# SkyTNT/midi-model

Hardware: AMD Instinct MI355X
Metric: MIDI events/sec, training step (fwd+bwd+clip+AdamW), tv2o-medium, seq=2048 (higher is better)
Workload: dtype bf16; 1 GPU; tv2o-medium bf16 training step, per-GPU batch 16 x 2048 events x 8 tokens (BASELINE.json configs[1]); random-init weights, synthetic events; global_batch=16, seq_len=2048, parallelism=dp1, accumulate_grad_batches=1, optimizer=AdamW bf16-true + global-norm clip 1.0

## Files before the change

include/midihip.h:

```cpp
#ifndef MIDIHIP_H
#define MIDIHIP_H
#include <stdint.h>
#ifdef __cplusplus
extern "C" {
#endif

#define MH_F32 0
#define MH_BF16 1

#define MH_OK 0
#define MH_ERR_ARG (-1)
#define MH_ERR_LAUNCH (-2)
#define MH_ERR_UNSUPPORTED (-3)

const char* mh_last_error(void);
int mh_version(void);
int mh_ab_builds(void);
int mh_set_option(const char* name, int value);
int mh_get_option(const char* name);

int mh_gemm_nt(const void* A, int64_t lda, const void* B, int64_t ldb, void* C, int64_t ldc, const void* R,
               int64_t ldr, int64_t M, int64_t N, int64_t K, float alpha, float beta, int dtype, int splitk,
               void* workspace, void* stream);
int mh_gemm(const void* A, int64_t lda, int transA, const void* B, int64_t ldb, int transB, void* C, int64_t ldc,
            const void* R, int64_t ldr, int64_t M, int64_t N, int64_t K, float alpha, float beta, int dtype, int splitk,
            void* workspace, void* stream);
int mh_gemm_swiglu(const void* A, int64_t lda, const void* W, int64_t ldw, void* GU, int64_t ldgu, void* ACT,
                   int64_t ldact, int64_t M, int64_t I, int64_t K, int dtype, void* stream);
int mh_gemm_rope(const void* A, int64_t lda, const void* W, int64_t ldw, void* C, int64_t ldc, const void* table,
                 int64_t npos, int64_t S, int64_t pos0, int head_dim, int64_t M, int64_t N, int64_t K, int dtype, void* stream);
int mh_gemm_dswiglu(const void* A, int64_t lda, const void* B, int64_t ldb, const void* GU, int64_t ldgu, void* DGU,
                    int64_t lddgu, int64_t M, int64_t I, int64_t K, int dtype, void* stream);
int mh_gemm_rowss(const void* A, int64_t lda, const void* B, int64_t ldb, void* C, int64_t ldc, const void* R, int64_t ldr,
                  float* rowss, int64_t M, int64_t N, int64_t K, int dtype, void* stream);
int mh_row_rstd(const void* x, int64_t ldx, const float* parts, int nparts, int64_t M, int D, float eps, float* rstd, int dtype,
                void* stream);
int mh_gemm_rope_scaled(const void* A, int64_t lda, const void* W, int64_t ldw, void* C, int64_t ldc, const void* table,
                        int64_t npos, int64_t S, int64_t pos0, int head_dim, const float* rowscale, int64_t M, int64_t N, int64_t K,
                        int dtype, void* stream);
int mh_gemm_swiglu_scaled(const void* A, int64_t lda, const void* W, int64_t ldw, void* GU, int64_t ldgu, void* ACT, int64_t ldact,
                          const float* rowscale, int64_t M, int64_t I, int64_t K, int dtype, void* stream);
int mh_gemm_nt_scaled(const void* A, int64_t lda, const void* B, int64_t ldb, void* C, int64_t ldc, const float* rowscale, int64_t M,
                      int64_t N, int64_t K, int dtype, void* stream);
int mh_gemm_dswiglu_scaled(const void* A, int64_t lda, const void* B, int64_t ldb, const void* GU, int64_t ldgu, void* DGU,
                           int64_t lddgu, const float* rowscale, int64_t M, int64_t I, int64_t K, int dtype, void* stream);
int mh_splitk_fold_blocks(int64_t M);
int mh_gemm_splitk_reduce_fold(const void* workspace, void* C, int64_t ldc, const void* R, int64_t ldr, int64_t M, int64_t N,
                               int splitk, float alpha, float beta, const void* wnorm, const void* W, int64_t ldw, float* colpart,
                               int dtype, void* stream);
int mh_rmsnorm_bwd_folded(const void* x, const float* rstd, const void* t, const void* dres, void* dx, int64_t M, int D, int dtype,
                          void* stream);
int mh_scale_cols(const void* W, int64_t ldw, const void* w, void* out, int64_t ldo, int64_t Nr, int K, int dtype, void* stream);
int mh_scale_cols_batched(const int64_t* jobs, int njobs, int K, int dtype, void* stream);
int mh_gemm_splitk_reduce(const void* workspace, void* C, int64_t ldc, const void* R, int64_t ldr, int64_t M,
                          int64_t N, int splitk, float alpha, float beta, int dtype, void* stream);
#define MH_SKINNY_PLAIN 0
#define MH_SKINNY_GATEUP 1
int mh_gemm_skinny(const void* A, int64_t lda, const void* W, int64_t ldw, void* C, int64_t ldc, const void* R,
                   int64_t ldr, int mode, float norm_eps, const int64_t* row_ids, const int64_t* res_ids, int64_t M,
                   int64_t N, int64_t K, int dtype, void* stream);
int mh_gemm_skinny_wide(const void* A, int64_t lda, const void* W, int64_t ldw, void* C, int64_t ldc, const void* R,
                        int64_t ldr, int mode, float norm_eps, const int64_t* row_ids, const int64_t* res_ids, int64_t M,
                        int64_t N, int64_t K, int dtype, void* stream);
int mh_transpose(const void* in, int64_t ldi, void* out, int64_t ldo, int64_t rows, int64_t cols, int dtype,
                 void* stream);

int mh_embed_sum_fwd(const int64_t* tok, const void* table, void* out, int64_t M, int T, int64_t V, int D,
                     int dtype, void* stream);
int mh_concat_tok_fwd(const void* hidden, const int64_t* tok, int64_t ldtok, const void* table, void* out,
                      int64_t M, int T, int64_t V, int D, int dtype, void* stream);
int mh_embed_scatter_bwd(const int64_t* tok, int64_t ldtok, int T, const void* dout, int rows_per_m, int jstride,
                         int j0, float* dtable_f32, int64_t M, int64_t V, int D, int64_t pad_id, int dtype,
                         void* stream);
int mh_embed_segment_bwd(const int64_t* src_rows, const int64_t* seg_start, const void* dout, int64_t ld,
                         float* dtable_f32, int64_t V, int D, int64_t n_occ, int64_t pad_id, int dtype, void* stream);
int mh_embed_segment_sum(const int64_t* src_rows, const int64_t* seg_start, const void* rows, int64_t ld, float* sum_f32,
                         int64_t ldsum, int64_t V, int D, int64_t n_occ, int dtype, void* stream);
int mh_embed_split_hi_lo(const float* s, void* hi, void* lo, int64_t n, int dtype, void* stream);
int mh_embed_table_norm_bwd(const void* t_hi, const void* t_lo, const void* e, const float* rstd, float* acc32, int64_t V, int D,
                            int64_t pad_id, int dtype, void* stream);
int mh_token_segments_chunk(void);
int mh_token_segments(const int64_t* tok, int64_t ldtok, int64_t n_rows, int n_cols, int64_t V, int64_t row_mul,
                      int64_t col_mul, int64_t add, int64_t* src_rows, int64_t* seg_start, int32_t* work, void* stream);
int mh_cast_from_f32(const float* src, void* dst, int64_t n, int accumulate, int dtype, void* stream);
int mh_copy_rows(const void* src, int64_t src_ld, void* dst, int64_t dst_ld, int64_t M, int D, int accumulate,
                 int dtype, void* stream);

int mh_collate_windows(const int16_t* tokens, int64_t n_events, const int64_t* win_start, const int64_t* win_len,
// ... 133 lines not shown
```

midi-model_amd/csrc/common.h:

```cpp
#pragma once
#include <hip/hip_runtime.h>
#include <stdint.h>

#include "../../include/midihip.h"

#define MH_WAVE 64

typedef __bf16 bf16;
typedef __attribute__((ext_vector_type(8))) __bf16 bf16x8;
typedef __attribute__((ext_vector_type(4))) __bf16 bf16x4;
typedef __attribute__((ext_vector_type(4))) float f32x4;
typedef __attribute__((ext_vector_type(16))) float f32x16;
typedef __attribute__((address_space(3))) void lds_void_t;
typedef __attribute__((address_space(1))) const void glb_void_t;

void mh_set_error(const char* fmt, ...);
#define MH_REQUIRE(cond, ...)            \
  do {                                   \
    if (!(cond)) {                       \
      mh_set_error(__VA_ARGS__);         \
      return MH_ERR_ARG;                 \
    }                                    \
  } while (0)
#define MH_LAUNCH_CHECK()                                            \
// ... 137 lines not shown
  auto take = [&](uint32_t ohi, uint32_t olo) {
    const bool better = ohi > hi || (ohi == hi && olo > lo);
    hi = better ? ohi : hi;
    lo = better ? olo : lo;
  };
  take(dpp_move_u<0xB1>(hi), dpp_move_u<0xB1>(lo));
  take(dpp_move_u<0x4E>(hi), dpp_move_u<0x4E>(lo));
  take(dpp_move_u<0x141>(hi), dpp_move_u<0x141>(lo));
  take(dpp_move_u<0x140>(hi), dpp_move_u<0x140>(lo));
  {
    auto a = __builtin_amdgcn_permlane16_swap(hi, hi, false, false);
    auto b = __builtin_amdgcn_permlane16_swap(lo, lo, false, false);
    hi = a[0];
    lo = b[0];
    take(a[1], b[1]);
  }
  {
    auto a = __builtin_amdgcn_permlane32_swap(hi, hi, false, false);
    auto b = __builtin_amdgcn_permlane32_swap(lo, lo, false, false);
    hi = a[0];
    lo = b[0];
    take(a[1], b[1]);
  }
  return ((uint64_t)hi << 32) | lo;
}

__device__ inline int lds_swz(int row) { return (((row >> 1) & 1) << 2) | (((row >> 2) & 1) << 1) | ((row >> 3) & 1); }
__device__ inline int lds_tile_off(int row, int chunk) { return row * 128 + ((chunk ^ lds_swz(row)) << 4); }

__device__ inline void glds16(const void* src, void* lds_rows8) {
  __builtin_amdgcn_global_load_lds((glb_void_t*)src, (lds_void_t*)lds_rows8, 16, 0, 0);
}

__device__ inline void gemm_tile_of(int idx, int tiles_m, int tiles_n, int GM, int& tm, int& tn) {
  const int width = GM * tiles_n;
  const int gid = idx / width;
  const int first = gid * GM;
  const int gsize = (tiles_m - first < GM) ? tiles_m - first : GM;
  const int rem = idx - gid * width;
  tn = rem / gsize;
  tm = first + (rem - tn * gsize);
}

__device__ inline int pi32(int i) { return (i & ~12) | ((i & 4) << 1) | ((i & 8) >> 1); }
```

midi-model_amd/csrc/gemm_pp256.hip:

```cpp
#include <limits.h>

#include <type_traits>

#include "common.h"

namespace {

__device__ __attribute__((aligned(16))) char g_zero16[16];

constexpr int QBM = 256, QBN = 256, QBK = 32;
constexpr int OP_BYTES = 256 * 64;
constexpr int STAGE_BYTES = 2 * OP_BYTES;
constexpr int NSTAGE = 4;
constexpr int LDS_BYTES = NSTAGE * STAGE_BYTES;
constexpr int NWAVE = 8;
constexpr int NI = 2;

typedef __attribute__((ext_vector_type(4))) short s16x4_t;

__device__ inline int tswz(int krow) { return (krow & 3) | ((krow >> 1) & 4); }
__device__ inline int xswz(int row) { return (0x1230 >> (((row >> 2) & 3) * 4)) & 3; }

struct StageCtx {
  const bf16* p[NI];
// ... 265 lines not shown
    for (int p = 0; p < 2; ++p) {
      stamp();
      if (2 * t + p > 0) mfma_phase(p ^ 1);
      else stamp();
      bar();
      stamp();
      load_slot(t, p, steady);
      wait_next(2 * t + p, steady);
      bar();
    }
  };

#pragma unroll
  for (int s = 0; s < LA; ++s)
    if (s < nreg) issue(s);
  if (nt > 0) wait_out((nreg < LA ? nreg : LA) - need(0));
  bar();
  mark(253);
  const int nsteady = nt > 2 ? nt - 2 : 0;
  if (grp == 0) {
    for (int t = 0; t < nsteady; ++t) tile_g0(t, std::true_type{});
    for (int t = nsteady; t < nt; ++t) tile_g0(t, std::false_type{});
  } else {
    for (int t = 0; t < nsteady; ++t) tile_g1(t, std::true_type{});
    for (int t = nsteady; t < nt; ++t) tile_g1(t, std::false_type{});
    if (nt > 0) mfma_phase(1);
  }
  mark(254);
  if constexpr (TL) {
    asm volatile("s_waitcnt lgkmcnt(0)" ::: "memory");
  }
}

template <bool TA, bool TB, int ABL, int EPI, int ML, int NRM>
__global__ __launch_bounds__(512, 2) void gemm_pp256_kernel(const bf16* __restrict__ A, int64_t lda,
                                                            const bf16* __restrict__ B, int64_t ldb, bf16* C, int64_t ldc,
                                                            const bf16* R, int64_t ldr, int64_t M, int64_t N, int64_t K,
                                                            float alpha, float beta, int tiles_n, int nwg,
                                                            int64_t k_per_split, float* __restrict__ ws,
                                                            const void* __restrict__ zero16, float* aux, int lean_epi) {
  static_assert(NRM == 0 || (ML == 1 && ABL == 0 && !TA && (!TB || (EPI == 1 && NRM == 2))), "the norm forms ride on the K-step-64 loops only");
  static_assert(NRM != 1 || EPI == 0, "sum-of-squares partials come out of the plain epilogue");
  extern __shared__ __attribute__((aligned(16))) char smem[];
  const int tid = threadIdx.x, lane = tid & 63;
  const int wave = __builtin_amdgcn_readfirstlane(tid >> 6);
  const int grp = wave >> 2;
  const int wn = wave & 3;

  const int nitems = nwg * (int)gridDim.z;
  const int lin = blockIdx.x + nwg * (int)blockIdx.z;
  const int q = nitems >> 3, r8 = nitems & 7, xcd = lin & 7;
  const int item = (xcd < r8 ? xcd * (q + 1) : r8 * (q + 1) + (xcd - r8) * q) + (lin >> 3);
  const int zslice = item / nwg;
  int tm, tn;
  gemm_tile_of(item - zslice * nwg, nwg / tiles_n, tiles_n, 4, tm, tn);
  const int64_t m0 = (int64_t)tm * QBM, n0 = (int64_t)tn * (EPI == 2 ? 128 : QBN);

  const int64_t kbeg = (int64_t)zslice * k_per_split;
  const int64_t kend = (kbeg + k_per_split < K) ? kbeg + k_per_split : K;

  f32x4 acc[4][8];
#pragma unroll
  for (int a = 0; a < 4; ++a)
#pragma unroll
    for (int b = 0; b < 8; ++b) acc[a][b] = f32x4{0.f, 0.f, 0.f, 0.f};
  const int fi = lane & 15, fg = lane >> 4;
  auto bar = [&]() {
    __builtin_amdgcn_sched_barrier(0);
    __builtin_amdgcn_s_barrier();
    __builtin_amdgcn_sched_barrier(0);
  };

  if constexpr (ML >= 1) {
    if constexpr (NRM == 2) {
      if (wave == 0) {
        const int64_t r = m0 + lane * 4;
        glds16((r + 4 <= M) ? (const void*)(aux + r) : zero16, smem + LDS_BYTES);
      }
    }
    p8_main_loop<EPI, ABL, TB>(smem, A, lda, B, ldb, M, N, m0, n0, kbeg, kend, wave, lane, zero16, acc);
    if constexpr ((ABL & 128) != 0) {
      __syncthreads();
      if (blockIdx.x == 0 && blockIdx.z == 0)
        for (int i = tid; i < P8_DBG_BYTES / 8; i += 512)
          reinterpret_cast<uint64_t*>(ws)[i] = reinterpret_cast<const uint64_t*>(smem + 2 * P8_BUF)[i];
      __syncthreads();
    }
  } else {
// ... 410 lines not shown
          const bf16x2 lo = __builtin_convertvector(f32x2{a4[0], a4[1]}, bf16x2), hi2 = __builtin_convertvector(f32x2{a4[2], a4[3]}, bf16x2);
          f32x4 r4;
          r4[0] = (float)lo[0];
          r4[1] = (float)lo[1];
          r4[2] = (float)hi2[0];
          r4[3] = (float)hi2[1];
          *reinterpret_cast<f32x4*>(wreg + row * 256 + ((ch ^ (row & 15)) << 4)) = r4;
        }
      if (half == 0) request(1);
#pragma unroll
      for (int i = 0; i < 8; ++i) {
        const int row = i * 8 + lrow;
        const f32x4 lo = *reinterpret_cast<const f32x4*>(wreg + row * 256 + (((2 * c) ^ (row & 15)) << 4));
        const f32x4 hi = *reinterpret_cast<const f32x4*>(wreg + row * 256 + (((2 * c + 1) ^ (row & 15)) << 4));
        const int64_t m = m0 + grp * 128 + half * 64 + row;
        float v[8] = {lo[0], lo[1], lo[2], lo[3], hi[0], hi[1], hi[2], hi[3]};
        if (rot) {
          const int pc = c ^ 4;
          const f32x4 plo = *reinterpret_cast<const f32x4*>(wreg + row * 256 + (((2 * pc) ^ (row & 15)) << 4));
          const f32x4 phi = *reinterpret_cast<const f32x4*>(wreg + row * 256 + (((2 * pc + 1) ^ (row & 15)) << 4));
          const float pv[8] = {plo[0], plo[1], plo[2], plo[3], phi[0], phi[1], phi[2], phi[3]};
          float cf[8], sf[8];
          expand8_bf16(cv[i], cf);
          expand8_bf16(sv[i], sf);
#pragma unroll
          for (int e = 0; e < 8; ++e) v[e] = __builtin_fmaf(v[e], cf[e], pv[e] * sf[e]);
        }
        if (m >= M || n + 8 > N) continue;
        __builtin_nontemporal_store(cvt8_bf16(v), reinterpret_cast<bf16x8*>(C + m * ldc + n));
      }
    }
    return;
  }
  const bool use_r = (R != nullptr && beta != 0.f);
  const bool line_ok = !partial && (ldc & 7) == 0 && ((uintptr_t)C & 15) == 0 &&
                       (!use_r || ((ldr & 7) == 0 && ((uintptr_t)R & 15) == 0));
  if (lean_epi && line_ok && m0 + QBM <= M && n0 + QBN <= N && ldc < (1 << 22) && ldr < (1 << 22)) {
    char* wreg = smem + wave * 16384;
    const int lrow = lane >> 3, c = lane & 7;
    const __amdgpu_buffer_rsrc_t rc = tile_rsrc(C + m0 * ldc + n0 + wn * 64, (255 * ldc + 64) * 2);
    const __amdgpu_buffer_rsrc_t rr = tile_rsrc(use_r ? R + m0 * ldr + n0 + wn * 64 : nullptr, use_r ? (255 * ldr + 64) * 2 : 0);
    const unsigned vo_c = (unsigned)(((grp * 128 + lrow) * (int)ldc + c * 8) * 2), so_c = (unsigned)ldc * 16u;
    const unsigned vo_r = (unsigned)(((grp * 128 + lrow) * (int)ldr + c * 8) * 2), so_r = (unsigned)ldr * 16u;
    float* auxp = nullptr;
    if constexpr (NRM == 1) auxp = aux + ((n0 + wn * 64) >> 6) * M + m0 + grp * 128 + lrow;
    auto turn = [&](auto with_r) {
    constexpr bool use_r = decltype(with_r)::value;
    bf16x8 rv[2][8];
    if (use_r) {
#pragma unroll
      for (int half = 0; half < 2; ++half)
#pragma unroll
        for (int i = 0; i < 8; ++i)
          rv[half][i] = as_bf16x8(__builtin_amdgcn_raw_buffer_load_b128(rr, vo_r, (unsigned)(half * 8 + i) * so_r, 0));
    }
#pragma unroll
    for (int half = 0; half < 2; ++half) {
#pragma unroll
      for (int fmh = 0; fmh < 4; ++fmh)
#pragma unroll
        for (int fn = 0; fn < 4; ++fn) {
          const int row = fmh * 16 + fi, ch = fn * 4 + fg;
          f32x4 t4 = acc[fn][half * 4 + fmh];
          if constexpr (NRM == 2) t4 *= rs[half * 4 + fmh];
          *reinterpret_cast<f32x4*>(wreg + row * 256 + ((ch ^ (row & 15)) << 4)) = t4;
        }
// ... 125 lines not shown
          *reinterpret_cast<f32x4*>(dst) = v;
        } else {
          for (int e = 0; e < 4 && n + e < N; ++e) dst[e] = v[e];
        }
        continue;
      }
      if (vec_ok && n + 3 < N) {
        if (R != nullptr && beta != 0.f) {
          bf16x4 rv = *reinterpret_cast<const bf16x4*>(R + m * ldr + n);
#pragma unroll
          for (int e = 0; e < 4; ++e) v[e] = alpha * v[e] + beta * (float)rv[e];
        } else {
#pragma unroll
          for (int e = 0; e < 4; ++e) v[e] = alpha * v[e];
        }
        bf16x4 o;
#pragma unroll
        for (int e = 0; e < 4; ++e) o[e] = (bf16)v[e];
        *reinterpret_cast<bf16x4*>(C + m * ldc + n) = o;
      } else {
        for (int e = 0; e < 4 && n + e < N; ++e) {
          float x = alpha * v[e];
          if (R != nullptr && beta != 0.f) x += beta * (float)R[m * ldr + n + e];
          C[m * ldc + n + e] = (bf16)x;
        }
      }
    }
  }
}

}
extern thread_local int g_mh_gemm_lean_epi;
namespace {
template <bool TA, bool TB, int ABL, int EPI = 0, int ML = 0, int NRM = 0>
int launch_one(const void* A, int64_t lda, const void* B, int64_t ldb, void* C, int64_t ldc, const void* R, int64_t ldr,
               int64_t M, int64_t N, int64_t K, float alpha, float beta, int splitk, void* workspace, hipStream_t st,
               float* aux = nullptr) {
  constexpr int LDSB = LDS_BYTES + ((ABL & 128) ? P8_DBG_BYTES : 0) + (NRM == 2 ? 1024 : 0);
  constexpr int MAX_DEV = 64;
  static void* zero16_of[MAX_DEV] = {};
  static bool attr_set_of[MAX_DEV] = {};
  int dev = 0;
  if (hipGetDevice(&dev) != hipSuccess || dev < 0 || dev >= MAX_DEV) {
    mh_set_error("gemm_pp256: no current device (or ordinal %d beyond %d)", dev, MAX_DEV - 1);
    return MH_ERR_LAUNCH;
  }
  void* zero16 = __atomic_load_n(&zero16_of[dev], __ATOMIC_ACQUIRE);
  if (zero16 == nullptr) {
    if (hipGetSymbolAddress(&zero16, HIP_SYMBOL(g_zero16)) != hipSuccess) {
      mh_set_error("gemm_pp256: hipGetSymbolAddress(g_zero16) failed");
      return MH_ERR_LAUNCH;
    }
    __atomic_store_n(&zero16_of[dev], zero16, __ATOMIC_RELEASE);
  }
  if (!__atomic_load_n(&attr_set_of[dev], __ATOMIC_ACQUIRE)) {
    hipError_t e = hipFuncSetAttribute(reinterpret_cast<const void*>(&gemm_pp256_kernel<TA, TB, ABL, EPI, ML, NRM>),
                                       hipFuncAttributeMaxDynamicSharedMemorySize, LDSB);
    if (e != hipSuccess) {
      mh_set_error("gemm_pp256: cannot raise dynamic LDS to %d bytes: %s", LDSB, hipGetErrorString(e));
      return MH_ERR_LAUNCH;
    }
    __atomic_store_n(&attr_set_of[dev], true, __ATOMIC_RELEASE);
  }
  const int64_t tiles_m = (M + QBM - 1) / QBM, tiles_n = (EPI == 2) ? N / 256 : (N + QBN - 1) / QBN;
  const int nwg = (int)(tiles_m * tiles_n);
  constexpr int KSTEP = (ML == 1) ? 64 : QBK;
  const int64_t kps = ((K + splitk - 1) / splitk + KSTEP - 1) / KSTEP * KSTEP;
  dim3 grid(nwg, 1, splitk);
  gemm_pp256_kernel<TA, TB, ABL, EPI, ML, NRM><<<grid, 512, LDSB, st>>>((const bf16*)A, lda, (const bf16*)B, ldb, (bf16*)C, ldc,
                                                          (const bf16*)R, ldr, M, N, K, alpha, beta, (int)tiles_n, nwg, kps,
                                                          (float*)workspace, zero16, aux, g_mh_gemm_lean_epi);
  MH_LAUNCH_CHECK();
  return MH_OK;
}

}

extern thread_local int g_mh_gemm_ablate;
extern thread_local int g_mh_gemm_k64;

int mh_gemm_pp256_bf16(const void* A, int64_t lda, int ta, const void* B, int64_t ldb, int tb, void* C, int64_t ldc,
                       const void* R, int64_t ldr, int64_t M, int64_t N, int64_t K, float alpha, float beta, int splitk,
                       void* workspace, hipStream_t st) {
#define MH_PP(TA_, TB_, ABL_) \
  return launch_one<TA_, TB_, ABL_>(A, lda, B, ldb, C, ldc, R, ldr, M, N, K, alpha, beta, splitk, workspace, st)
#ifndef MH_AB_BUILDS
  MH_REQUIRE(g_mh_gemm_ablate == 0, "gemm: option gemm_ablate = %d selects a micro-benchmark build, which is only in the A/B test "
             "library (libmidihip_ab.so)", g_mh_gemm_ablate);
#else
  MH_REQUIRE(g_mh_gemm_ablate != 128 || (workspace != nullptr && splitk == 1), "gemm_ablate 128 (timeline) needs a workspace and splitk 1");
  MH_REQUIRE(!(g_mh_gemm_k64 && !ta && !tb) || g_mh_gemm_ablate == 0 || g_mh_gemm_ablate == 1 || g_mh_gemm_ablate == 4 ||
                 g_mh_gemm_ablate == 128 || g_mh_gemm_ablate == 64,
             "gemm_ablate %d is not built for the K-step-64 main loop (set gemm_k64 = 0 for the K-step-32 ablations)", g_mh_gemm_ablate);
  if (ta == tb && g_mh_gemm_ablate && !(g_mh_gemm_k64 && !ta)) {
#define MH_AB(X_) \
  case X_:        \
    if (ta) MH_PP(true, true, X_); \
    MH_PP(false, false, X_);
    switch (g_mh_gemm_ablate) { MH_AB(1) MH_AB(3) MH_AB(4) MH_AB(5) MH_AB(8) MH_AB(12) MH_AB(32) default: break; }
#undef MH_AB
  }
  if (g_mh_gemm_ablate == 64) {
    if (ta && tb) MH_PP(true, true, 64);
    if (ta) MH_PP(true, false, 64);
    if (tb) MH_PP(false, true, 64);
    MH_PP(false, false, 64);
  }
#endif
  if (ta && tb) MH_PP(true, true, 0);
  if (ta) MH_PP(true, false, 0);
  if (tb && g_mh_gemm_k64 == 1)
// ... 68 lines not shown
```

midi-model_amd/engine.py:

```python
from __future__ import annotations

import math
from dataclasses import dataclass, field
from typing import Callable, List, NamedTuple, Optional

import os

import torch

from . import ops, tokfirst


@dataclass
class StackSpec:
    name: str
    D: int
    H: int
    I: int
    L: int
    eps: float
    theta: float
    kind: str

    @property
# ... 270 lines not shown
        ops.swiglu_bwd(keep.gu, da, dgu)
        del da
    linear_wgrad(dx, a, lg.wd, accumulate)
    del a
    dh2 = _empty((M, D), dx)
    ops.gemm_nt(dgu, lw.wgu, dh2, tb=True)
    linear_wgrad(dgu, keep.h2, lg.wgu, accumulate)
    del dgu
    dx2 = _empty((M, D), dx)
    ops.rmsnorm_bwd(keep.x2, lw.n2, keep.rstd2, dh2, dx, dx2, lg.n2, accumulate)
    do = dh2
    ops.gemm_nt(dx2, lw.wo, do, tb=True)
    linear_wgrad(dx2, keep.o, lg.wo, accumulate)
    dqkv = _empty((M, 3 * D), dx)
    if seqs is not None:
        ops.attn_bwd_seqs(keep.qkv, keep.o, do, keep.lse, dqkv, seqs, H, spec.scale, rope.cos, rope.sin)
    elif spec.kind == "event":
        ops.attn_bwd(keep.qkv, keep.o, do, keep.lse, dqkv, nseq, slen, H, spec.scale, rope.cos, rope.sin)
    else:
        ops.tokattn_bwd(keep.qkv, do, dqkv, nseq, slen, H, spec.scale, rope.cos, rope.sin)
    dh1 = do
    ops.gemm_nt(dqkv, lw.wqkv, dh1, tb=True)
    linear_wgrad(dqkv, keep.h1, lg.wqkv, accumulate)
    del dqkv
    ops.rmsnorm_bwd(keep.x, lw.n1, keep.rstd1, dh1, dx2, dx, lg.n1, accumulate)
    return dx


def layer_backward_folded(spec: StackSpec, lw: LayerTensors, lg: LayerTensors, fold, keep: LayerSaved, dx: torch.Tensor, nseq: int,
                          slen: int, rope: RopeTable, accumulate: bool, seqs=None) -> torch.Tensor:
    M, D = dx.shape
    H = spec.H
    wq_n, wgu_n = fold
    dx2, do = _folded_mlp_o_backward(spec, lw, lg, wgu_n, keep, dx, accumulate)
    dz1 = _empty((M, 3 * D), dx)
    if seqs is not None:
        ops.attn_bwd_seqs(keep.qkv, keep.o, do, keep.lse, dz1, seqs, H, spec.scale, rope.cos, rope.sin, rowscale=keep.rstd1)
    elif spec.kind == "event":
        ops.attn_bwd(keep.qkv, keep.o, do, keep.lse, dz1, nseq, slen, H, spec.scale, rope.cos, rope.sin, rowscale=keep.rstd1)
    else:
        ops.tokattn_bwd(keep.qkv, do, dz1, nseq, slen, H, spec.scale, rope.cos, rope.sin, rowscale=keep.rstd1)
    t1 = do
    ops.gemm_nt(dz1, wq_n, t1, tb=True)
    ops.wgrad_folded(dz1, keep.x, lg.wqkv, lw.n1, lw.wqkv, lg.n1, accumulate)
    del dz1
    ops.rmsnorm_bwd_folded(keep.x, keep.rstd1, t1, dx2, dx)
    return dx


def _folded_mlp_o_backward(spec: StackSpec, lw: LayerTensors, lg: LayerTensors, wgu_n: torch.Tensor, keep: LayerSaved,
                           dx: torch.Tensor, accumulate: bool):
    M, D = dx.shape
    I = spec.I
    a = keep.a
    if a is None:
        a = _empty((M, I), dx)
        ops.swiglu_fwd(keep.gu, a)
    dz2 = _empty((M, 2 * I), dx)
    ops.gemm_dswiglu(dx, lw.wd, keep.gu, dz2, rowscale=keep.rstd2)
    linear_wgrad(dx, a, lg.wd, accumulate)
    del a
    t2 = _empty((M, D), dx)
    ops.gemm_nt(dz2, wgu_n, t2, tb=True)
    ops.wgrad_folded(dz2, keep.x2, lg.wgu, lw.n2, lw.wgu, lg.n2, accumulate)
    del dz2
    dx2 = _empty((M, D), dx)
    ops.rmsnorm_bwd_folded(keep.x2, keep.rstd2, t2, dx, dx2)
    do = t2
    ops.gemm_nt(dx2, lw.wo, do, tb=True)
    linear_wgrad(dx2, keep.o, lg.wo, accumulate)
    return dx2, do


class TokFirstGrads(NamedTuple):
    dhidden: torch.Tensor
    dtable32: torch.Tensor


def tok_first_backward(spec: StackSpec, lw: LayerTensors, lg: LayerTensors, fold, keep: LayerSaved, first: tokfirst.TokFirst,
                       dx: torch.Tensor, nseq: int, rope: RopeTable, accumulate: bool) -> TokFirstGrads:
    M, D = dx.shape
    H, T = spec.H, tokfirst.TN
    N, V = first.hidden.shape[0], first.table.shape[0]
    assert N == nseq and M == N * T
    wq_n, wgu_n = fold
    xc, rstd_c, zc = keep.x, keep.rstd1, keep.qkv
    dres, do = _folded_mlp_o_backward(spec, lw, lg, wgu_n, keep, dx, accumulate)
    dz = _empty((M, 3 * D), dx)
    dzc = _empty((N + 2 * V, 3 * D), dx)
    tokfirst.tokattn_bwd_rows(zc, first.ids, N, V, do, dz, dzc[:N], rstd_c, N, H, spec.scale, rope.cos, rope.sin)
    del do
    src, seg, vseg, vstart = tokfirst.occurrence_lists(first.ids[:, : T - 1], V, T, 1)
    S = _empty((V, 3 * D), dx, torch.float32)
    tokfirst.segment_sum_fixed_order(src, vseg, vstart, dz, S)
    del dz
    tokfirst.split_hi_lo(S, dzc[N:N + V], dzc[N + V:])
    del S
    tc = _empty((N + 2 * V, D), dx)
    ops.gemm_nt(dzc, wq_n, tc, tb=True)
    ops.wgrad_folded(dzc, xc, lg.wqkv, lw.n1, lw.wqkv, lg.n1, accumulate)
    del dzc
    dres_h = _empty((N, D), dx)
    ops.copy_rows(dres, T * D, dres_h, D, N, D)
# ... 261 lines not shown
```

midi-model_amd/ops.py:

```python
from __future__ import annotations

from typing import Optional

import os
import threading

import torch

from .lib import MH_BF16, MH_F32, lib

_DT = {torch.float32: MH_F32, torch.bfloat16: MH_BF16}


def dt(t: torch.Tensor) -> int:
    try:
        return _DT[t.dtype]
    except KeyError:
        raise TypeError(f"unsupported dtype {t.dtype}: the HIP path computes in float32 or bfloat16") from None


def _stream() -> int:
    return torch.cuda.current_stream().cuda_stream


# ... 389 lines not shown
def scale_cols_jobs(triples) -> torch.Tensor:
    rows = []
    for W, w, out in triples:
        assert W.is_contiguous() and out.is_contiguous() and W.shape == out.shape and w.shape == (W.shape[1],)
        rows.append([W.data_ptr(), w.data_ptr(), out.data_ptr(), W.shape[0]])
    return torch.tensor(rows, dtype=torch.int64, device=triples[0][0].device)


def scale_cols_batched(jobs: torch.Tensor, K: int, like: torch.Tensor) -> None:
    lib().call("mh_scale_cols_batched", _p(jobs), jobs.shape[0], K, dt(like), _stream())


def gemm_nt_scaled(a: torch.Tensor, b: torch.Tensor, out: torch.Tensor, rowscale: torch.Tensor) -> torch.Tensor:
    M, N = out.shape
    K = a.shape[1]
    assert b.shape == (N, K) and a.shape[0] == M and rowscale.shape == (M,) and rowscale.dtype == torch.float32
    prof = gemm_profile
    if prof is not None:
        e0, e1 = torch.cuda.Event(enable_timing=True), torch.cuda.Event(enable_timing=True)
        e0.record()
    lib().call("mh_gemm_nt_scaled", _p(a), _rowmajor(a), _p(b), _rowmajor(b), _p(out), _rowmajor(out), _p(rowscale), M, N, K,
               dt(a), _stream())
    if prof is not None:
        e1.record()
        prof.append((e0, e1, 2.0 * M * N * K, (M, N, K, 1, 0, 0, "+rowscale")))
    return out


def wgrad_folded(dz: torch.Tensor, x: torch.Tensor, dw: torch.Tensor, wnorm: torch.Tensor, W: torch.Tensor,
                 dnorm: torch.Tensor, accumulate: bool) -> None:
    M = dz.shape[0]
    N, K = dw.shape
    assert dz.shape[1] == N and x.shape == (M, K) and W.shape == (N, K) and wnorm.shape == (K,) and dnorm.shape == (K,)
    splitk = max(2, _pick_splitk(N, K, M))
    ws = torch.empty((splitk, N, K), dtype=torch.float32, device=dw.device)
    prof = gemm_profile
    if prof is not None:
        e0, e1 = torch.cuda.Event(enable_timing=True), torch.cuda.Event(enable_timing=True)
        e0.record()
    lib().call("mh_gemm", _p(dz), _rowmajor(dz), 1, _p(x), _rowmajor(x), 1, _p(dw), _rowmajor(dw), None, 0, N, K, M, 1.0, 0.0,
               dt(dw), splitk, _p(ws), _stream())
    nblk = lib().cdll.mh_splitk_fold_blocks(N)
    colpart = torch.empty((nblk, K), dtype=torch.float32, device=dw.device)
    lib().call("mh_gemm_splitk_reduce_fold", _p(ws), _p(dw), _rowmajor(dw), _p(dw) if accumulate else None, _rowmajor(dw) if accumulate else 0,
               N, K, splitk, 1.0, 1.0 if accumulate else 0.0, _p(wnorm), _p(W), _rowmajor(W), _p(colpart), dt(dw), _stream())
    lib().call("mh_colsum", _p(colpart), nblk, _p(dnorm), K, int(accumulate), dt(dnorm), _stream())
    if prof is not None:
        e1.record()
        prof.append((e0, e1, 2.0 * M * N * K, (N, K, M, splitk, 1, 1, "+fold")))


def rope_(qkv: torch.Tensor, cos_t: torch.Tensor, sin_t: torch.Tensor, S: int, pos0: int, H: int, hd: int, direction: int = 1):
    M = qkv.shape[0]
    assert qkv.is_contiguous() and qkv.shape[1] == 3 * H * hd
    assert cos_t.shape[0] >= pos0 + min(S, M), "RoPE table too short"
    lib().call("mh_rope", _p(qkv), _p(cos_t), _p(sin_t), M, S, pos0, H, hd, direction, dt(qkv), _stream())
    return qkv


def attn_fwd(qkv, o, lse, B: int, S: int, H: int, scale: float):
    vt = None
    if qkv.dtype == torch.bfloat16 and (_attn_v3() & 17) != 17:
        Sp = round_up(S, 64)
        vt = torch.empty((B * H * 64 * Sp,), dtype=qkv.dtype, device=qkv.device)
        lib().call("mh_attn_prep_fwd", _p(qkv), _p(vt), B, S, H, dt(qkv), _stream())
    lib().call("mh_attn_fwd", _p(qkv), _p(vt), _p(o), _p(lse), B, S, H, scale, dt(qkv), _stream())
# ... 2 lines not shown

def attn_bwd_scaled_ok(qkv: torch.Tensor) -> bool:
    return qkv.dtype == torch.bfloat16 and (_attn_v3() & 46) == 46


def attn_bwd(qkv, o, dout, lse, dqkv, B: int, S: int, H: int, scale: float, cos_t=None, sin_t=None, rowscale=None):
    Sp = round_up(S, 64)
    v3 = _attn_v3()
    fused = qkv.dtype == torch.bfloat16 and (v3 & 14) == 14 and (v3 & 32) != 0
    delta = torch.empty(((2 if fused else 1) * B * H * Sp,), dtype=torch.float32, device=qkv.device)
    if rowscale is not None:
        assert fused and rowscale.shape == (B * S,) and rowscale.dtype == torch.float32 and rowscale.is_contiguous()
        lib().call("mh_attn_bwd_o_scaled", _p(qkv), _p(o), _p(dout), _p(lse), _p(delta), _p(dqkv), _p(rowscale), B, S, H, scale,
                   _p(cos_t), _p(sin_t), dt(qkv), _stream())
        return dqkv
    if fused:
        lib().call("mh_attn_bwd_o", _p(qkv), _p(o), _p(dout), _p(lse), _p(delta), _p(dqkv), B, S, H, scale, _p(cos_t), _p(sin_t),
                   dt(qkv), _stream())
        return dqkv
    qt = kt = dot = None
    if qkv.dtype == torch.bfloat16 and (v3 & 14) != 14:
        n = B * H * 64 * Sp
        buf = torch.empty((3, n), dtype=qkv.dtype, device=qkv.device)
        qt, kt, dot = buf[0], buf[1], buf[2]
    lib().call("mh_attn_prep_bwd", _p(qkv), _p(o), _p(dout), _p(delta), _p(qt), _p(kt), _p(dot), B, S, H, dt(qkv), _stream())
    lib().call("mh_attn_bwd", _p(qkv), _p(dout), _p(lse), _p(delta), _p(qt), _p(kt), _p(dot), _p(dqkv), B, S, H, scale,
               _p(cos_t), _p(sin_t), dt(qkv), _stream())
    return dqkv


_PACKED = ("SeqPlan", "attn_seq_plan", "rope_pos_", "attn_fwd_seqs", "attn_bwd_seqs",
           "kv_append_rows", "attn_decode_rows", "attn_decode_append_rows", "kv_store_seqs")
_WIDE = ("gemm_skinny_wide", "skinny_wide_ok", "decode_wide_enabled")


def __getattr__(name: str):
    if name in _PACKED:
        from . import ops_packed
        return getattr(ops_packed, name)
    if name in _WIDE:
        from . import ops_wide
        return getattr(ops_wide, name)
    raise AttributeError(f"module {__name__!r} has no attribute {name!r}")


def tokattn_fwd(qkv, o, N: int, T: int, H: int, scale: float, cos_t=None, sin_t=None):
    lib().call("mh_tokattn_fwd", _p(qkv), _p(o), N, T, H, scale, _p(cos_t), _p(sin_t), dt(qkv), _stream())
    return o


def tokattn_bwd(qkv, dout, dqkv, N: int, T: int, H: int, scale: float, cos_t=None, sin_t=None, rowscale=None):
    if rowscale is not None:
        assert rowscale.shape == (N * T,) and rowscale.dtype == torch.float32 and rowscale.is_contiguous()
        lib().call("mh_tokattn_bwd_scaled", _p(qkv), _p(dout), _p(dqkv), _p(rowscale), N, T, H, scale, _p(cos_t), _p(sin_t),
                   dt(qkv), _stream())
        return dqkv
    lib().call("mh_tokattn_bwd", _p(qkv), _p(dout), _p(dqkv), N, T, H, scale, _p(cos_t), _p(sin_t), dt(qkv), _stream())
    return dqkv


def swiglu_fwd(gu, a):
    M, I2 = gu.shape
    lib().call("mh_swiglu_fwd", _p(gu), _p(a), M, I2 // 2, dt(gu), _stream())
    return a


def swiglu_bwd(gu, da, dgu):
    M, I2 = gu.shape
    lib().call("mh_swiglu_bwd", _p(gu), _p(da), _p(dgu), M, I2 // 2, dt(gu), _stream())
# ... 102 lines not shown
```

Before: 360,100 events/s.

## Group per-layer weight-gradient GEMMs into one launch with fused norm-fold epilogue

Adds a grouped variant of the pp256 GEMM kernel that computes up to eight weight-gradient problems (wd, wgu, wo, wqkv) of one layer in a single launch, with a problem table and XCD-aware tile mapping. The grouped kernel's epilogue folds the RMSNorm weight scaling and column partial sums directly, replacing the split-K workspace plus a separate reduce-fold pass. The event-layer backward defers its wgrad calls and issues them together after the attention backward. The aim is to cut launch count and fp32 split-K workspace traffic and to fill the GPU with tiles from several GEMMs at once. In exchange there is no split-K, so long contractions (M=32768) run on fewer tiles per problem, and weight-gradient work is delayed until later in the layer backward.

```diff
diff --git a/include/midihip.h b/include/midihip.h
--- a/include/midihip.h
+++ b/include/midihip.h
@@ -54,6 +54,20 @@
 int mh_scale_cols_batched(const int64_t* jobs, int njobs, int K, int dtype, void* stream);
 int mh_gemm_splitk_reduce(const void* workspace, void* C, int64_t ldc, const void* R, int64_t ldr, int64_t M,
                           int64_t N, int splitk, float alpha, float beta, int dtype, void* stream);
+typedef struct {
+  const void* dz;  int64_t lddz;
+  const void* x;   int64_t ldx;
+  void* dw;        int64_t lddw;
+  const void* R;   int64_t ldr;
+  int64_t N, K_out;
+  float alpha, beta;
+  const void* wnorm;
+  const void* W;   int64_t ldw;
+  float* colpart;
+} mh_wgrad_problem;
+int mh_wgrad_grouped_fold_blocks(int64_t N);
+int mh_gemm_wgrad_grouped(const mh_wgrad_problem* p, int n, int64_t Kc, int dtype, void* stream);
+int mh_wgrad_grouped_item(const mh_wgrad_problem* p, int n, int lin, int* problem, int* tm, int* tn);
 #define MH_SKINNY_PLAIN 0
 #define MH_SKINNY_GATEUP 1
 int mh_gemm_skinny(const void* A, int64_t lda, const void* W, int64_t ldw, void* C, int64_t ldc, const void* R,
diff --git a/midi-model_amd/csrc/common.h b/midi-model_amd/csrc/common.h
--- a/midi-model_amd/csrc/common.h
+++ b/midi-model_amd/csrc/common.h
@@ -193,7 +193,7 @@
   __builtin_amdgcn_global_load_lds((glb_void_t*)src, (lds_void_t*)lds_rows8, 16, 0, 0);
 }
 
-__device__ inline void gemm_tile_of(int idx, int tiles_m, int tiles_n, int GM, int& tm, int& tn) {
+__host__ __device__ inline void gemm_tile_of(int idx, int tiles_m, int tiles_n, int GM, int& tm, int& tn) {
   const int width = GM * tiles_n;
   const int gid = idx / width;
   const int first = gid * GM;
diff --git a/midi-model_amd/csrc/gemm_pp256.hip b/midi-model_amd/csrc/gemm_pp256.hip
--- a/midi-model_amd/csrc/gemm_pp256.hip
+++ b/midi-model_amd/csrc/gemm_pp256.hip
@@ -321,28 +321,80 @@
   }
 }
 
-template <bool TA, bool TB, int ABL, int EPI, int ML, int NRM>
+constexpr int GRP_MAX = 8;
+struct GrpProblem {
+  const bf16* A;
+  const bf16* B;
+  bf16* C;
+  const bf16* R;
+  const bf16* wnorm;
+  const bf16* W;
+  float* colpart;
+  int64_t lda, ldb, ldc, ldr, ldw, M, N;
+  float alpha, beta;
+  int tile0, tiles_n;
+};
+struct GrpTable {
+  GrpProblem p[GRP_MAX];
+  int n, nitems;
+};
+__host__ __device__ inline int xcd_item_of(int lin, int nitems) {
+  const int q = nitems >> 3, r8 = nitems & 7, xcd = lin & 7;
+  return (xcd < r8 ? xcd * (q + 1) : r8 * (q + 1) + (xcd - r8) * q) + (lin >> 3);
+}
+__host__ __device__ inline int grp_item_of(const GrpTable& t, int lin, int& tm, int& tn) {
+  const int item = xcd_item_of(lin, t.nitems);
+  int pi = 0;
+#pragma unroll
+  for (int j = 1; j < GRP_MAX; ++j)
+    if (j < t.n && item >= t.p[j].tile0) pi = j;
+  const int tiles_n = t.p[pi].tiles_n;
+  const int tiles_m = (int)((t.p[pi].M + QBM - 1) / QBM);
+  gemm_tile_of(item - t.p[pi].tile0, tiles_m, tiles_n, 4, tm, tn);
+  return pi;
+}
+template <bool GRP>
+struct GrpArg {
+  typedef int type;
+};
+template <>
+struct GrpArg<true> {
+  typedef GrpTable type;
+};
+
+template <bool TA, bool TB, int ABL, int EPI, int ML, int NRM, bool GRP = false>
 __global__ __launch_bounds__(512, 2) void gemm_pp256_kernel(const bf16* __restrict__ A, int64_t lda,
                                                             const bf16* __restrict__ B, int64_t ldb, bf16* C, int64_t ldc,
                                                             const bf16* R, int64_t ldr, int64_t M, int64_t N, int64_t K,
                                                             float alpha, float beta, int tiles_n, int nwg,
                                                             int64_t k_per_split, float* __restrict__ ws,
-                                                            const void* __restrict__ zero16, float* aux, int lean_epi) {
+                                                            const void* __restrict__ zero16, float* aux, int lean_epi,
+                                                            const typename GrpArg<GRP>::type gtab) {
   static_assert(NRM == 0 || (ML == 1 && ABL == 0 && !TA && (!TB || (EPI == 1 && NRM == 2))), "the norm forms ride on the K-step-64 loops only");
   static_assert(NRM != 1 || EPI == 0, "sum-of-squares partials come out of the plain epilogue");
+  static_assert(!GRP || (TA && TB && ABL == 0 && EPI == 0 && ML == 0 && NRM == 0), "the grouped launch is the weight-gradient form");
   extern __shared__ __attribute__((aligned(16))) char smem[];
   const int tid = threadIdx.x, lane = tid & 63;
   const int wave = __builtin_amdgcn_readfirstlane(tid >> 6);
   const int grp = wave >> 2;
   const int wn = wave & 3;
 
-  const int nitems = nwg * (int)gridDim.z;
-  const int lin = blockIdx.x + nwg * (int)blockIdx.z;
-  const int q = nitems >> 3, r8 = nitems & 7, xcd = lin & 7;
-  const int item = (xcd < r8 ? xcd * (q + 1) : r8 * (q + 1) + (xcd - r8) * q) + (lin >> 3);
-  const int zslice = item / nwg;
-  int tm, tn;
-  gemm_tile_of(item - zslice * nwg, nwg / tiles_n, tiles_n, 4, tm, tn);
+  int zslice = 0, tm, tn;
+  const bf16 *wnorm = nullptr, *Wf = nullptr;
+  float* colpart = nullptr;
+  int64_t ldw = 0;
+  if constexpr (GRP) {
+    const GrpProblem& P = gtab.p[grp_item_of(gtab, (int)blockIdx.x, tm, tn)];
+    A = P.A, lda = P.lda, B = P.B, ldb = P.ldb, C = P.C, ldc = P.ldc, R = P.R, ldr = P.ldr, M = P.M, N = P.N;
+    alpha = P.alpha, beta = P.beta;
+    wnorm = P.wnorm, Wf = P.W, ldw = P.ldw, colpart = P.colpart;
+  } else {
+    const int nitems = nwg * (int)gridDim.z;
+    const int lin = blockIdx.x + nwg * (int)blockIdx.z;
+    const int item = xcd_item_of(lin, nitems);
+    zslice = item / nwg;
+    gemm_tile_of(item - zslice * nwg, nwg / tiles_n, tiles_n, 4, tm, tn);
+  }
   const int64_t m0 = (int64_t)tm * QBM, n0 = (int64_t)tn * (EPI == 2 ? 128 : QBN);
 
   const int64_t kbeg = (int64_t)zslice * k_per_split;
@@ -819,6 +871,97 @@
     }
     return;
   }
+  if constexpr (GRP) {
+    if (wnorm != nullptr) {
+      char* wreg = smem + wave * 16384;
+      const int lrow = lane >> 3, c = lane & 7;
+      const int64_t n = n0 + wn * 64 + c * 8;
+      const bool n_ok = (n + 8 <= N);
+      float wnf[8], cs[8];
+#pragma unroll
+      for (int e = 0; e < 8; ++e) wnf[e] = cs[e] = 0.f;
+      if (n_ok) expand8_bf16(*reinterpret_cast<const bf16x8*>(wnorm + n), wnf);
+      auto turn = [&](auto with_r) {
+        constexpr bool WR = decltype(with_r)::value;
+        bf16x8 wq[2][8], rq[2][8];
+        auto request = [&](int half) {
+#pragma unroll
+          for (int i = 0; i < 8; ++i) {
+            const int64_t m = m0 + grp * 128 + half * 64 + i * 8 + lrow;
+            if (m < M && n_ok) {
+              wq[half][i] = *reinterpret_cast<const bf16x8*>(Wf + m * ldw + n);
+              if constexpr (WR) rq[half][i] = *reinterpret_cast<const bf16x8*>(R + m * ldr + n);
+            }
+          }
+        };
+#pragma unroll
+        for (int half = 0; half < 2; ++half) {
+#pragma unroll
+          for (int fmh = 0; fmh < 4; ++fmh)
+#pragma unroll
+            for (int fn = 0; fn < 4; ++fn) {
+              const int row = fmh * 16 + fi, ch = fn * 4 + fg;
+              *reinterpret_cast<f32x4*>(wreg + row * 256 + ((ch ^ (row & 15)) << 4)) = acc[fn][half * 4 + fmh];
+            }
+          if (half == 0) request(0);
+          if (half == (WR ? 1 : 0)) request(1);
+#pragma unroll
+          for (int i = 0; i < 8; ++i) {
+            const int row = i * 8 + lrow;
+            const f32x4 lo = *reinterpret_cast<const f32x4*>(wreg + row * 256 + (((2 * c) ^ (row & 15)) << 4));
+            const f32x4 hi = *reinterpret_cast<const f32x4*>(wreg + row * 256 + (((2 * c + 1) ^ (row & 15)) << 4));
+            const int64_t m = m0 + grp * 128 + half * 64 + row;
+            if (m >= M || !n_ok) continue;
+            float v[8] = {lo[0], lo[1], lo[2], lo[3], hi[0], hi[1], hi[2], hi[3]};
+            float wf[8];
+            expand8_bf16(wq[half][i], wf);
+#pragma unroll
+            for (int e = 0; e < 8; ++e) {
+              v[e] = alpha * v[e];
+              cs[e] += v[e] * wf[e];
+              v[e] *= wnf[e];
+            }
+            if constexpr (WR) {
+              float rf[8];
+              expand8_bf16(rq[half][i], rf);
+#pragma unroll
+              for (int e = 0; e < 8; ++e) v[e] += beta * rf[e];
+            }
+            bf16x8 o;
+#pragma unroll
+            for (int e = 0; e < 8; ++e) o[e] = (bf16)v[e];
+            __builtin_nontemporal_store(o, reinterpret_cast<bf16x8*>(C + m * ldc + n));
+          }
+        }
+      };
+      if (__builtin_amdgcn_readfirstlane((int)(R != nullptr && beta != 0.f))) turn(std::true_type{});
+      else turn(std::false_type{});
+#pragma unroll
+      for (int e = 0; e < 8; ++e) {
+        cs[e] += __shfl_xor(cs[e], 8);
+        cs[e] += __shfl_xor(cs[e], 16);
+        cs[e] += __shfl_xor(cs[e], 32);
+      }
+      f32x4* half_sums = reinterpret_cast<f32x4*>(smem + (wn + 4) * 16384) + c * 2;
+      if (grp == 1 && lrow == 0) {
+        half_sums[0] = f32x4{cs[0], cs[1], cs[2], cs[3]};
+        half_sums[1] = f32x4{cs[4], cs[5], cs[6], cs[7]};
+      }
+      __syncthreads();
+      if (grp == 0 && lrow == 0 && n_ok) {
+        f32x4 s0 = half_sums[0], s1 = half_sums[1];
+#pragma unroll
+        for (int e = 0; e < 4; ++e) {
+          s0[e] = cs[e] + s0[e];
+          s1[e] = cs[4 + e] + s1[e];
+        }
+        float* dst = colpart + (int64_t)tm * N + n;
+        *reinterpret_cast<f32x4*>(dst) = s0;
+        *reinterpret_cast<f32x4*>(dst + 4) = s1;
+      }
+      return;
+    }
+  }
   const bool use_r = (R != nullptr && beta != 0.f);
   const bool line_ok = !partial && (ldc & 7) == 0 && ((uintptr_t)C & 15) == 0 &&
                        (!use_r || ((ldr & 7) == 0 && ((uintptr_t)R & 15) == 0));
@@ -1010,11 +1153,8 @@
 }
 extern thread_local int g_mh_gemm_lean_epi;
 namespace {
-template <bool TA, bool TB, int ABL, int EPI = 0, int ML = 0, int NRM = 0>
-int launch_one(const void* A, int64_t lda, const void* B, int64_t ldb, void* C, int64_t ldc, const void* R, int64_t ldr,
-               int64_t M, int64_t N, int64_t K, float alpha, float beta, int splitk, void* workspace, hipStream_t st,
-               float* aux = nullptr) {
-  constexpr int LDSB = LDS_BYTES + ((ABL & 128) ? P8_DBG_BYTES : 0) + (NRM == 2 ? 1024 : 0);
+template <auto KERNEL>
+int launch_prepare(int LDSB, void** zero16_out) {
   constexpr int MAX_DEV = 64;
   static void* zero16_of[MAX_DEV] = {};
   static bool attr_set_of[MAX_DEV] = {};
@@ -1032,14 +1172,24 @@
     __atomic_store_n(&zero16_of[dev], zero16, __ATOMIC_RELEASE);
   }
   if (!__atomic_load_n(&attr_set_of[dev], __ATOMIC_ACQUIRE)) {
-    hipError_t e = hipFuncSetAttribute(reinterpret_cast<const void*>(&gemm_pp256_kernel<TA, TB, ABL, EPI, ML, NRM>),
-                                       hipFuncAttributeMaxDynamicSharedMemorySize, LDSB);
+    hipError_t e = hipFuncSetAttribute(reinterpret_cast<const void*>(KERNEL), hipFuncAttributeMaxDynamicSharedMemorySize, LDSB);
     if (e != hipSuccess) {
       mh_set_error("gemm_pp256: cannot raise dynamic LDS to %d bytes: %s", LDSB, hipGetErrorString(e));
       return MH_ERR_LAUNCH;
     }
     __atomic_store_n(&attr_set_of[dev], true, __ATOMIC_RELEASE);
   }
+  *zero16_out = zero16;
+  return MH_OK;
+}
+
+template <bool TA, bool TB, int ABL, int EPI = 0, int ML = 0, int NRM = 0>
+int launch_one(const void* A, int64_t lda, const void* B, int64_t ldb, void* C, int64_t ldc, const void* R, int64_t ldr,
+               int64_t M, int64_t N, int64_t K, float alpha, float beta, int splitk, void* workspace, hipStream_t st,
+               float* aux = nullptr) {
+  constexpr int LDSB = LDS_BYTES + ((ABL & 128) ? P8_DBG_BYTES : 0) + (NRM == 2 ? 1024 : 0);
+  void* zero16 = nullptr;
+  if (int rc = launch_prepare<&gemm_pp256_kernel<TA, TB, ABL, EPI, ML, NRM>>(LDSB, &zero16)) return rc;
   const int64_t tiles_m = (M + QBM - 1) / QBM, tiles_n = (EPI == 2) ? N / 256 : (N + QBN - 1) / QBN;
   const int nwg = (int)(tiles_m * tiles_n);
   constexpr int KSTEP = (ML == 1) ? 64 : QBK;
@@ -1047,14 +1197,86 @@
   dim3 grid(nwg, 1, splitk);
   gemm_pp256_kernel<TA, TB, ABL, EPI, ML, NRM><<<grid, 512, LDSB, st>>>((const bf16*)A, lda, (const bf16*)B, ldb, (bf16*)C, ldc,
                                                           (const bf16*)R, ldr, M, N, K, alpha, beta, (int)tiles_n, nwg, kps,
-                                                          (float*)workspace, zero16, aux, g_mh_gemm_lean_epi);
+                                                          (float*)workspace, zero16, aux, g_mh_gemm_lean_epi, 0);
   MH_LAUNCH_CHECK();
   return MH_OK;
 }
 
-}
-
+void grp_table_of(const mh_wgrad_problem* p, int n, GrpTable& t) {
+  t.n = n;
+  int tile0 = 0;
+  for (int j = 0; j < GRP_MAX; ++j) {
+    GrpProblem& g = t.p[j];
+    if (j >= n) {
+      g = GrpProblem{};
+      g.tile0 = INT_MAX;
+      continue;
+    }
+    g.A = (const bf16*)p[j].dz, g.lda = p[j].lddz, g.B = (const bf16*)p[j].x, g.ldb = p[j].ldx;
+    g.C = (bf16*)p[j].dw, g.ldc = p[j].lddw, g.R = (const bf16*)p[j].R, g.ldr = p[j].ldr;
+    g.wnorm = (const bf16*)p[j].wnorm, g.W = (const bf16*)p[j].W, g.ldw = p[j].ldw, g.colpart = p[j].colpart;
+    g.M = p[j].N, g.N = p[j].K_out, g.alpha = p[j].alpha, g.beta = p[j].beta;
+    g.tile0 = tile0;
+    g.tiles_n = (int)((g.N + QBN - 1) / QBN);
+    tile0 += (int)((g.M + QBM - 1) / QBM) * g.tiles_n;
+  }
+  t.nitems = tile0;
+}
+
+int grp_validate(const mh_wgrad_problem* p, int n, int64_t Kc, int dtype) {
+  MH_REQUIRE(dtype == MH_BF16, "gemm_wgrad_grouped: bf16 only");
+  MH_REQUIRE(p != nullptr && n >= 1 && n <= GRP_MAX && Kc > 0, "gemm_wgrad_grouped: 1 to %d problems and a contraction length (n=%d Kc=%ld)",
+             GRP_MAX, n, (long)Kc);
+  int64_t tiles = 0;
+  for (int j = 0; j < n; ++j) {
+    const mh_wgrad_problem& q = p[j];
+    MH_REQUIRE(q.N > 0 && q.K_out > 0 && q.dz != nullptr && q.x != nullptr && q.dw != nullptr, "gemm_wgrad_grouped: problem %d is empty", j);
+    MH_REQUIRE(q.lddz % 8 == 0 && q.ldx % 8 == 0 && q.lddz >= q.N && q.ldx >= q.K_out && q.lddw >= q.K_out,
+               "gemm_wgrad_grouped: problem %d: leading dimensions must be multiples of 8 elements and cover the rows", j);
+    MH_REQUIRE((((uintptr_t)q.dz | (uintptr_t)q.x) & 15) == 0, "gemm_wgrad_grouped: problem %d: dz / x must be 16-byte aligned", j);
+    MH_REQUIRE(q.beta == 0.f || (q.R != nullptr && q.ldr >= q.K_out), "gemm_wgrad_grouped: problem %d: beta != 0 needs R", j);
+    if (q.wnorm != nullptr) {
+      MH_REQUIRE(q.W != nullptr && q.colpart != nullptr && q.K_out % 8 == 0 && q.lddw % 8 == 0 && q.ldw % 8 == 0 && q.ldw >= q.K_out &&
+                     (q.R == nullptr || q.ldr % 8 == 0),
+                 "gemm_wgrad_grouped: problem %d: the fold epilogue needs W, colpart and whole 16-byte lines (K_out, lddw, ldw, ldr %% 8 == 0)", j);
+      MH_REQUIRE((((uintptr_t)q.dw | (uintptr_t)q.W | (uintptr_t)q.wnorm | (uintptr_t)q.R | (uintptr_t)q.colpart) & 15) == 0,
+                 "gemm_wgrad_grouped: problem %d: the fold epilogue needs 16-byte aligned dw, W, wnorm, R and colpart", j);
+    }
+    tiles += ((q.N + QBM - 1) / QBM) * ((q.K_out + QBN - 1) / QBN);
+  }
+  MH_REQUIRE(tiles < (1ll << 30), "gemm_wgrad_grouped: too many tiles");
+  return MH_OK;
+}
+
+}
+
+extern thread_local int g_mh_gemm_variant;
 extern thread_local int g_mh_gemm_ablate;
+
+extern "C" int mh_wgrad_grouped_fold_blocks(int64_t N) { return (int)(N < 1 ? 1 : (N + QBM - 1) / QBM); }
+
+extern "C" int mh_gemm_wgrad_grouped(const mh_wgrad_problem* p, int n, int64_t Kc, int dtype, void* stream) {
+  if (int rc = grp_validate(p, n, Kc, dtype)) return rc;
+  MH_REQUIRE(g_mh_gemm_variant != 0 && g_mh_gemm_ablate == 0, "gemm_wgrad_grouped: served by the production bf16 kernel only");
+  GrpTable t;
+  grp_table_of(p, n, t);
+  void* zero16 = nullptr;
+  if (int rc = launch_prepare<&gemm_pp256_kernel<true, true, 0, 0, 0, 0, true>>(LDS_BYTES, &zero16)) return rc;
+  const int64_t kps = (Kc + QBK - 1) / QBK * QBK;
+  gemm_pp256_kernel<true, true, 0, 0, 0, 0, true><<<dim3(t.nitems, 1, 1), 512, LDS_BYTES, (hipStream_t)stream>>>(
+      nullptr, 0, nullptr, 0, nullptr, 0, nullptr, 0, 0, 0, Kc, 1.f, 0.f, 0, t.nitems, kps, nullptr, zero16, nullptr, g_mh_gemm_lean_epi, t);
+  MH_LAUNCH_CHECK();
+  return MH_OK;
+}
+
+extern "C" int mh_wgrad_grouped_item(const mh_wgrad_problem* p, int n, int lin, int* problem, int* tm, int* tn) {
+  if (p == nullptr || n < 1 || n > GRP_MAX) return -1;
+  GrpTable t;
+  grp_table_of(p, n, t);
+  if (lin >= 0 && lin < t.nitems && problem != nullptr && tm != nullptr && tn != nullptr) *problem = grp_item_of(t, lin, *tm, *tn);
+  return t.nitems;
+}
+
 extern thread_local int g_mh_gemm_k64;
 
 int mh_gemm_pp256_bf16(const void* A, int64_t lda, int ta, const void* B, int64_t ldb, int tb, void* C, int64_t ldc,
diff --git a/midi-model_amd/engine.py b/midi-model_amd/engine.py
--- a/midi-model_amd/engine.py
+++ b/midi-model_amd/engine.py
@@ -326,7 +326,11 @@
     M, D = dx.shape
     H = spec.H
     wq_n, wgu_n = fold
-    dx2, do = _folded_mlp_o_backward(spec, lw, lg, wgu_n, keep, dx, accumulate)
+    I = spec.I
+    pend = None
+    if spec.kind == "event" and seqs is None and ops.wgrad_grouped_ok([(D, I), (2 * I, D), (D, D), (3 * D, D)], M, dx):
+        pend = []
+    dx2, do = _folded_mlp_o_backward(spec, lw, lg, wgu_n, keep, dx, accumulate, pend)
     dz1 = _empty((M, 3 * D), dx)
     if seqs is not None:
         ops.attn_bwd_seqs(keep.qkv, keep.o, do, keep.lse, dz1, seqs, H, spec.scale, rope.cos, rope.sin, rowscale=keep.rstd1)
@@ -336,14 +340,19 @@
         ops.tokattn_bwd(keep.qkv, do, dz1, nseq, slen, H, spec.scale, rope.cos, rope.sin, rowscale=keep.rstd1)
     t1 = do
     ops.gemm_nt(dz1, wq_n, t1, tb=True)
-    ops.wgrad_folded(dz1, keep.x, lg.wqkv, lw.n1, lw.wqkv, lg.n1, accumulate)
+    if pend is not None:
+        pend.append((dz1, keep.x, lg.wqkv, (lw.n1, lw.wqkv, lg.n1)))
+        ops.wgrad_grouped(pend, accumulate)
+        pend.clear()
+    else:
+        ops.wgrad_folded(dz1, keep.x, lg.wqkv, lw.n1, lw.wqkv, lg.n1, accumulate)
     del dz1
     ops.rmsnorm_bwd_folded(keep.x, keep.rstd1, t1, dx2, dx)
     return dx
 
 
 def _folded_mlp_o_backward(spec: StackSpec, lw: LayerTensors, lg: LayerTensors, wgu_n: torch.Tensor, keep: LayerSaved,
-                           dx: torch.Tensor, accumulate: bool):
+                           dx: torch.Tensor, accumulate: bool, pend: Optional[list] = None):
     M, D = dx.shape
     I = spec.I
     a = keep.a
@@ -352,17 +361,26 @@
         ops.swiglu_fwd(keep.gu, a)
     dz2 = _empty((M, 2 * I), dx)
     ops.gemm_dswiglu(dx, lw.wd, keep.gu, dz2, rowscale=keep.rstd2)
-    linear_wgrad(dx, a, lg.wd, accumulate)
+    if pend is not None:
+        pend.append((dx, a, lg.wd, None))
+    else:
+        linear_wgrad(dx, a, lg.wd, accumulate)
     del a
     t2 = _empty((M, D), dx)
     ops.gemm_nt(dz2, wgu_n, t2, tb=True)
-    ops.wgrad_folded(dz2, keep.x2, lg.wgu, lw.n2, lw.wgu, lg.n2, accumulate)
+    if pend is not None:
+        pend.append((dz2, keep.x2, lg.wgu, (lw.n2, lw.wgu, lg.n2)))
+    else:
+        ops.wgrad_folded(dz2, keep.x2, lg.wgu, lw.n2, lw.wgu, lg.n2, accumulate)
     del dz2
     dx2 = _empty((M, D), dx)
     ops.rmsnorm_bwd_folded(keep.x2, keep.rstd2, t2, dx, dx2)
     do = t2
     ops.gemm_nt(dx2, lw.wo, do, tb=True)
-    linear_wgrad(dx2, keep.o, lg.wo, accumulate)
+    if pend is not None:
+        pend.append((dx2, keep.o, lg.wo, None))
+    else:
+        linear_wgrad(dx2, keep.o, lg.wo, accumulate)
     return dx2, do
 
 
diff --git a/midi-model_amd/ops.py b/midi-model_amd/ops.py
--- a/midi-model_amd/ops.py
+++ b/midi-model_amd/ops.py
@@ -445,6 +445,11 @@
     M = dz.shape[0]
     N, K = dw.shape
     assert dz.shape[1] == N and x.shape == (M, K) and W.shape == (N, K) and wnorm.shape == (K,) and dnorm.shape == (K,)
+    if _pick_splitk(N, K, M) == 1:
+        from . import ops_grouped
+        if ops_grouped.wgrad_grouped_operands_ok([(dz, x, dw, (wnorm, W, dnorm))]):
+            ops_grouped.wgrad_grouped([(dz, x, dw, (wnorm, W, dnorm))], accumulate)
+            return
     splitk = max(2, _pick_splitk(N, K, M))
     ws = torch.empty((splitk, N, K), dtype=torch.float32, device=dw.device)
     prof = gemm_profile
@@ -513,9 +518,13 @@
 _PACKED = ("SeqPlan", "attn_seq_plan", "rope_pos_", "attn_fwd_seqs", "attn_bwd_seqs",
            "kv_append_rows", "attn_decode_rows", "attn_decode_append_rows", "kv_store_seqs")
 _WIDE = ("gemm_skinny_wide", "skinny_wide_ok", "decode_wide_enabled")
+_GROUPED = ("wgrad_grouped", "wgrad_grouped_ok", "wgrad_grouped_operands_ok", "wgrad_grouped_enabled", "wgrad_grouped_launches")
 
 
 def __getattr__(name: str):
+    if name in _GROUPED:
+        from . import ops_grouped
+        return getattr(ops_grouped, name)
     if name in _PACKED:
         from . import ops_packed
         return getattr(ops_packed, name)
diff --git a/midi-model_amd/ops_grouped.py b/midi-model_amd/ops_grouped.py
--- /dev/null
+++ b/midi-model_amd/ops_grouped.py
@@ -0,0 +1,85 @@
+from __future__ import annotations
+
+import ctypes
+import os
+
+import torch
+
+from . import ops
+from .lib import MH_BF16, lib
+from .ops import _p, _rowmajor, _stream, dt
+
+
+class _WgradProblem(ctypes.Structure):
+    _fields_ = [("dz", ctypes.c_void_p), ("lddz", ctypes.c_int64), ("x", ctypes.c_void_p), ("ldx", ctypes.c_int64),
+                ("dw", ctypes.c_void_p), ("lddw", ctypes.c_int64), ("R", ctypes.c_void_p), ("ldr", ctypes.c_int64),
+                ("N", ctypes.c_int64), ("K_out", ctypes.c_int64), ("alpha", ctypes.c_float), ("beta", ctypes.c_float),
+                ("wnorm", ctypes.c_void_p), ("W", ctypes.c_void_p), ("ldw", ctypes.c_int64), ("colpart", ctypes.c_void_p)]
+
+
+WGRAD_GROUP_MAX = 8
+wgrad_grouped_launches = 0
+
+
+def wgrad_grouped_enabled() -> bool:
+    return os.environ.get("MH_WGRAD_GROUPED", "1") != "0"
+
+
+def wgrad_grouped_operands_ok(problems) -> bool:
+    if not (1 <= len(problems) <= WGRAD_GROUP_MAX) or ops.get_option("gemm") == 0 or not wgrad_grouped_enabled():
+        return False
+    Kc = problems[0][0].shape[0]
+    for dz, x, dw, fold in problems:
+        if not (dz.is_cuda and dz.dtype == x.dtype == dw.dtype == torch.bfloat16 and dz.shape[0] == x.shape[0] == Kc):
+            return False
+        if _rowmajor(dz) % 8 or _rowmajor(x) % 8 or (dz.data_ptr() | x.data_ptr()) % 16:
+            return False
+        if fold is not None:
+            wnorm, W, _ = fold
+            if dw.shape[1] % 8 or _rowmajor(dw) % 8 or _rowmajor(W) % 8 or (dw.data_ptr() | W.data_ptr() | wnorm.data_ptr()) % 16:
+                return False
+    return True
+
+
+def wgrad_grouped_ok(shapes, Kc: int, like: torch.Tensor) -> bool:
+    if not like.is_cuda or like.dtype != torch.bfloat16 or ops.get_option("gemm") == 0 or not wgrad_grouped_enabled():
+        return False
+    if not (1 <= len(shapes) <= WGRAD_GROUP_MAX) or Kc < 1:
+        return False
+    tiles = sum(((n + 255) // 256) * ((k + 255) // 256) for n, k in shapes)
+    empty = -tiles % 256
+    return empty * 10 <= 256
+
+
+def wgrad_grouped(problems, accumulate: bool) -> None:
+    global wgrad_grouped_launches
+    assert wgrad_grouped_operands_ok(problems), "wgrad_grouped: bf16 problems over one contraction length on the production GEMM"
+    M = problems[0][0].shape[0]
+    arr = (_WgradProblem * len(problems))()
+    folds, flops, rows = [], 0.0, 0
+    for q, (dz, x, dw, fold) in zip(arr, problems):
+        N, K = dw.shape
+        assert dz.shape == (M, N) and x.shape == (M, K), (dz.shape, x.shape, dw.shape)
+        q.dz, q.lddz, q.x, q.ldx, q.dw, q.lddw = _p(dz), _rowmajor(dz), _p(x), _rowmajor(x), _p(dw), _rowmajor(dw)
+        q.R, q.ldr = (_p(dw), _rowmajor(dw)) if accumulate else (None, 0)
+        q.N, q.K_out, q.alpha, q.beta = N, K, 1.0, 1.0 if accumulate else 0.0
+        if fold is not None:
+            wnorm, W, dnorm = fold
+            assert W.shape == (N, K) and wnorm.shape == (K,) and dnorm.shape == (K,)
+            nblk = lib().cdll.mh_wgrad_grouped_fold_blocks(N)
+            colpart = torch.empty((nblk, K), dtype=torch.float32, device=dw.device)
+            q.wnorm, q.W, q.ldw, q.colpart = _p(wnorm), _p(W), _rowmajor(W), _p(colpart)
+            folds.append((colpart, nblk, dnorm, K))
+        flops += 2.0 * M * N * K
+        rows += N
+    prof = ops.gemm_profile
+    if prof is not None:
+        e0, e1 = torch.cuda.Event(enable_timing=True), torch.cuda.Event(enable_timing=True)
+        e0.record()
+    lib().call("mh_gemm_wgrad_grouped", arr, len(problems), M, MH_BF16, _stream())
+    for colpart, nblk, dnorm, K in folds:
+        lib().call("mh_colsum", _p(colpart), nblk, _p(dnorm), K, int(accumulate), dt(dnorm), _stream())
+    wgrad_grouped_launches += 1
+    if prof is not None:
+        e1.record()
+        prof.append((e0, e1, flops, (rows, max(p[2].shape[1] for p in problems), M, 1, 1, 1, "+grouped")))
```

Result: faster. 365,700 events/s (median of 6 runs) (+1.6%).
